# liuQuan98/GCL

Measured on AMD Instinct MI355X. Metric: active voxels/sec thru ResUNetBN2C fwd+bwd+GCL loss, KITTI 0.3m, higher is better.
Workload: dtype f32; 1 GPU; configs[2]: GCL training step (finest_contrastive_loss), ResUNetBN2C-32 conv1 k=5, KITTI-shaped ray-cast clouds @0.3 m, bs=4 x 7 clouds per GPU, positive groups 'fixed16'; global_batch=4, parallelism=dp1

## Files before the change

gcl_amd/MinkowskiEngine/native.py:

```python
import ctypes
import os
import threading

import torch
from torch.autograd.function import once_differentiable

from .. import _lib

PLAN_ENABLED = os.environ.get("GCL_PLAN", "1") == "1"
AUX_STREAM = {"0": "", "1": "1", "low": "low", "high": "high"}[os.environ.get("GCL_PLAN_AUX", "low")]


def _addr(t):
    return t.data_ptr() if t is not None else 0


_SIDE_STREAMS = {}


def eval_side_stream(device, n_rows=None):
    if os.environ.get("GCL_EVAL_SPLIT_MAPS", "1") == "0":
        return None
    if n_rows is not None and n_rows < int(os.environ.get("GCL_EVAL_SPLIT_MIN_ROWS", "100000")):
        return None
# ... 127 lines not shown
        if not self.handle:
            raise ValueError(lib.gcl_last_error().decode())
        self.handle = ctypes.c_void_p(self.handle)
        self._state = None
        self._key = None
        self.grad_targets = None
        self.bucket_of_param = None
        self.on_bucket = None
        self._param_ptrs = self._bn_ptrs = None
        self._ptr_key = None
        self.profile_next = False
        self.last_profile = None
        self._anchor = None
        self._aux = None
        self._eval_key = None

    def __del__(self):
        h, self.handle = getattr(self, "handle", None), None
        if h:
            try:
                _lib.load().gcl_plan_destroy(h)
            except Exception:
                pass

    @classmethod
    def from_tape(cls, tape, model, x_in, in_level, spec_keys):
        from . import ops
        if ops.PRECISION != "fp16x3" or not ops.FUSE_GRAD_ADD:
            raise ValueError("the plan runs the default arithmetic (fp16x3, fused gradient adds) only")
        params = [p for p in model.parameters()]
# ... 217 lines not shown
        for i, r in enumerate(self.records):
            for k in ("w", "bias", "bn_w", "bn_b"):
                p = r[k]
                if p >= 0 and p in self.bucket_of_param:
                    b = self.bucket_of_param[p]
                    lowest[b] = min(lowest.get(b, i), i)
        cuts = sorted(set(lowest.values()), reverse=True)
        segs, hi = [], n
        for c in cuts:
            segs.append((c, hi, sorted(b for b, i in lowest.items() if i == c)))
            hi = c
        if hi > 0:
            segs.append((0, hi, []))
        return segs

    def _backward(self, run, dy):
        lib = _lib.load()
        targets = run.grad_targets
        flat = None
        if targets is None:
            sizes = [p.numel() for p in self.params]
            flat = torch.empty(sum(sizes), dtype=torch.float32, device=dy.device)
            targets, off = [], 0
            for p, s in zip(self.params, sizes):
                targets.append(flat[off:off + s].view_as(p))
                off += s
        gp = (ctypes.c_void_p * len(targets))(*[t.data_ptr() for t in targets])
        st = _lib.stream()
        for first, last, buckets in run.segments:
            _lib.check(lib.gcl_plan_backward(self.handle, _lib.ptr(run.arena), _lib.ptr(dy, torch.float32), gp, first,
                                             last, st), "gcl_plan_backward")
            for b in buckets:
                self.on_bucket(b)
        if self.profile_next:
            self.profile_next = False
            self._profile_pending = True
            lib.gcl_plan_profile(self.handle, 0)
        run.done = True
        run.arena = run.maps = run.y = run.x = None
        return None if flat is None else targets

    def profile_records(self):
        lib = _lib.load()
        buf = (ctypes.c_double * (8 * 1024))()
        n = lib.gcl_plan_profile_read(self.handle, buf, 1024)
        return [tuple(buf[8 * i + j] for j in range(8)) for i in range(max(0, n))]
```

gcl_amd/_lib.py:

```python
import ctypes
import os
import subprocess

import torch

_HERE = os.path.dirname(os.path.abspath(__file__))
CSRC = os.path.join(_HERE, "csrc")
LIB_PATH = os.environ.get("GCL_LIB_PATH", os.path.join(CSRC, "libgcl_hip.so"))
SOURCES = ["coords.hip", "conv.hip", "norm.hip", "loss.hip", "pairloss.hip", "data.hip", "sc2pcr.hip", "plan.hip", "match.hip", "ransac.hip", "regstats.hip", "fpfh.hip",
           "valpose.hip", "pairmatch.hip", "icp.hip"]
HEADER = os.path.join(os.path.dirname(_HERE), "include", "gcl_amd.h")

_vp, _i32, _i64, _f32 = ctypes.c_void_p, ctypes.c_int32, ctypes.c_int64, ctypes.c_float
_f64 = ctypes.c_double

MAX_LEVELS, MAX_MAPS = 8, 16
MAPS_PINNED_BYTES = 512 * (MAX_MAPS + 1)
ERR_ARENA = -4


class MapSpec(ctypes.Structure):
    _fields_ = [("t_in", _i32), ("kernel_size", _i32), ("stride", _i32), ("tables", _i32), ("pairs", _i32)]


# ... 105 lines not shown
    "gcl_col_sum": (_i32, [_vp, _i64, _i32, _vp, _vp, _vp]),
    "gcl_maps_arena_bytes": (_i64, [_i64, _vp, _i32, _i32]),
    "gcl_maps_build": (_i32, [_vp, _i64, _vp, _i32, _i32, _vp, _i64, _vp, _vp, _vp]),
    "gcl_maps_build_split": (_i32, [_vp, _i64, _vp, _i32, _i32, _vp, _i64, _vp, _vp, _vp, _vp]),
    "gcl_plan_create": (_vp, [_vp, _i32, _i32, _i32, _vp, _i32, _i32]),
    "gcl_plan_destroy": (None, [_vp]),
    "gcl_plan_state_bytes": (_i64, [_vp]),
    "gcl_plan_arena_bytes": (_i64, [_vp, _vp]),
    "gcl_plan_forward": (_i32, [_vp, _vp, _vp, _vp, _vp, _vp, _vp, _i64, _vp, _vp]),
    "gcl_plan_eval_state_bytes": (_i64, [_vp]),
    "gcl_plan_eval_arena_bytes": (_i64, [_vp, _vp]),
    "gcl_plan_forward_eval": (_i32, [_vp, _vp, _vp, _vp, _vp, _i32, _vp, _vp, _i64, _vp, _vp]),
    "gcl_plan_backward": (_i32, [_vp, _vp, _vp, _vp, _i32, _i32, _vp]),
    "gcl_plan_release": (_i32, [_vp, _vp]),
    "gcl_plan_set_aux_stream": (_i32, [_vp, _vp]),
    "gcl_stream_create_cu_share": (_i32, [_i32, _i32, ctypes.POINTER(ctypes.c_void_p)]),
    "gcl_stream_destroy": (_i32, [_vp]),
    "gcl_plan_profile": (_i32, [_vp, _i32]),
    "gcl_plan_profile_read": (_i32, [_vp, _vp, _i32]),
    "gcl_sc2_chunks": (_i32, []),
    "gcl_sc2_refine_partial_len": (_i32, []),
    "gcl_sc2_confidence": (_i32, [_vp, _vp, _i32, _f32, _i32, _vp, _vp, _vp, _vp]),
    "gcl_sc2_confidence_scratch_bytes": (_i64, [_i32]),
    "gcl_sc2_confidence_sparse": (_i32, [_vp, _vp, _i32, _f32, _i32, _vp, _vp, _vp, _vp, _vp]),
    "gcl_sc2_register_scratch_bytes": (_i64, [_i32]),
    "gcl_sc2_register": (_i32, [_vp, _vp, _i32, _f32, _i32, _f32, _i32, _i32, _i32, _f32, _f32, _i32, _vp, _vp, _vp, _vp, _vp,
                                _vp, _vp, _vp, _vp, _vp]),
    "gcl_sc2_register_batch_scratch_bytes": (_i64, [_i32, _i32]),
    "gcl_sc2_register_batch": (_i32, [_vp, _vp, _i32, _i32, _vp, _vp, _f32, _i32, _f32, _i32, _i32, _f32, _f32, _i32, _vp, _vp,
                                      _vp, _vp, _vp, _vp, _vp, _vp, _vp, _vp]),
# ... 163 lines not shown
```

gcl_amd/csrc/plan.hip:

```cpp
#include "common.h"

#include <string.h>

#include <new>
#include <utility>
#include <vector>

namespace gcl {

__device__ __forceinline__ float amax4p(float m, const float4& v) {
  return fmaxf(m, fmaxf(fmaxf(fabsf(v.x), fabsf(v.y)), fmaxf(fabsf(v.z), fabsf(v.w))));
}
__device__ __forceinline__ void publish_amax_wg(float m, int* slot) {
#pragma unroll
  for (int o = 32; o > 0; o >>= 1) m = fmaxf(m, __shfl_xor(m, o));
  __shared__ float wm[4];
  if ((threadIdx.x & 63) == 0) wm[threadIdx.x >> 6] = m;
  __syncthreads();
  if (threadIdx.x == 0)
    amax_slot_publish(slot, __float_as_int(fmaxf(fmaxf(wm[0], wm[1]), fmaxf(wm[2], wm[3]))), blockIdx.x);
}

__global__ void __launch_bounds__(256) k_relu_fwd(const float4* __restrict__ x, long long n4, float4* __restrict__ y,
                                                  int* amax) {
// ... 66 lines not shown
    const int q = (int)(i - r * c4);
    float4 u = reinterpret_cast<const float4*>(a + r * a_ld)[q];
    if (b) {
      const float4 v = reinterpret_cast<const float4*>(b + r * b_ld)[q];
      u = make_float4(u.x + v.x, u.y + v.y, u.z + v.z, u.w + v.w);
    }
    y[i] = u;
  }
}
__global__ void __launch_bounds__(256) k_add2(const float4* __restrict__ a, const float4* __restrict__ b, long long n4,
                                              float4* __restrict__ y) {
  for (long long i = (long long)blockIdx.x * 256 + threadIdx.x; i < n4; i += (long long)gridDim.x * 256) {
    const float4 u = a[i], v = b[i];
    y[i] = make_float4(u.x + v.x, u.y + v.y, u.z + v.z, u.w + v.w);
  }
}
__global__ void __launch_bounds__(256) k_identity_pairs(int* __restrict__ p, long long n, long long total) {
  long long i = (long long)blockIdx.x * 256 + threadIdx.x;
  if (i < total) p[i] = i < n ? (int)i : -1;
}

void fill32(void* p, long long n_words, unsigned v, hipStream_t st);
void tables_fill(int64_t* tables, long long slots, int32_t* zero4, hipStream_t st);
int coords_insert_impl(const int32_t* coords, int64_t n, int64_t* table, int64_t cap, int32_t* status, bool table_ready,
                       void* stream);
int stride_map_impl(const int32_t* coords_in, int64_t n_in, const int32_t* n_in_dev, int32_t t_out, int64_t* table_out,
                    int64_t cap_out, int32_t* scratch, int32_t* coords_out, int32_t* n_out_dev, int32_t* status,
                    int64_t* index_out, bool table_ready, void* stream);

static inline unsigned grid_for(long long items, unsigned cap = 4096) {
// ... 284 lines not shown
  std::vector<long long> wK, wcin, wcout, off_fwd, off_bwd;
  long long bytes_fwd = 0, bytes_bwd = 0, wgs_fwd = 0, wgs_bwd = 0;
  int n_bwd = 0;
  std::vector<char> made;
  std::vector<char> fuse_relu;
  std::vector<int> cat_left;
  std::vector<int> mask_from;
  std::vector<long long> host_tables, uploaded;
  bool eval = false;
  void* const* bn_eval = nullptr;
  bool eval_repack = true;
  hipStream_t aux = nullptr;
  std::vector<hipEvent_t> events;
  size_t events_used = 0;
  bool aux_dirty = false;
  bool profile = false;
  std::vector<ProfRec> prof;
  size_t prof_used = 0;
};

static long long state_words(const Plan& P) { return (long long)P.worder.size() * (2 + 8 + 8); }

static int32_t* new_slot(Plan& P) {
  if (P.next_slot >= P.n_slots) {
    P.slots_exhausted = true;
    return P.slot_pool;
  }
  return P.slot_pool + (P.next_slot++) * GCL_AMAX_WORDS;
}

// ... 492 lines not shown
    float* scratch = A.take_n<float>(gcl_conv_bwd_weight_scratch_len(op.K, op.cin, op.cout, m.seg_off[op.K], n_sorted));
    const bool pl = pl_w;
    ProfScope ps(P, ws, 2, pairs, op.cin, op.cout, n_in, n_out, op.K);
    const int32_t* rgb = (sorted_side != 0 && n_sorted == m.n_out) ? m.dw_bounds : nullptr;
    PLAN_CALL(gcl_conv_bwd_weight_rg(pl ? (const float*)x.planes : x.ptr, n_in, pl ? (const float*)dy.planes : dy.ptr, n_out,
                                     pl ? 1 : 0, sorted_side, pa, pb, m.seg_off, op.K, op.cin, op.cout, 4, P.saved[i].x_amax,
                                     dy.amax, scratch, dW, rgb, (void*)ws));
  }
  if (op.bias >= 0) {
    double* scratch = A.take_n<double>(gcl_bn_scratch_len(n_out, op.cout));
    PLAN_CALL(gcl_col_sum(dy.ptr, n_out, op.cout, scratch, (float*)grads[op.bias], (void*)ws));
  }
  return GCL_OK;
}

static int plan_backward(Plan& P, const float* dy, void* const* grads, int first, int last, hipStream_t st) {
  Arena& A = P.A;
  const gcl_maps_desc& M = *P.maps;
  const size_t nw = P.worder.size();
  if (last == (int)P.ops.size()) {
    P.g[P.ops.back().y] = TState();
    P.g[P.ops.back().y].ptr = (float*)dy;
  }
  if (P.bwd_packed && last == (int)P.ops.size()) {
    int rcj = join_aux(P, st);
    if (rcj) return rcj;
  }
  if (!P.bwd_packed) {
    P.pack_bwd = (unsigned char*)A.take(P.bytes_bwd);
    if (P.n_bwd && !A.dry) {
      const long long* tab = (const long long*)P.state;
      PLAN_CALL(gcl_pack_weights_multi((const int64_t*)(tab + 2 * nw + 8 * nw), P.n_bwd, P.wgs_bwd, 4, P.w_amax, P.pack_bwd,
                                       (void*)st));
    }
    P.bwd_packed = true;
  }
  for (int i = last - 1; i >= first; --i) {
    const gcl_plan_op& op = P.ops[i];
    const long long n_out = M.n_rows[op.level_out], n_in = M.n_rows[op.level_in];
    TState g = P.g[op.y];
    P.g[op.y] = TState();
    if (!g.ptr) continue;
    int rc;
    switch (op.kind) {
      case GCL_OP_CONVBN: {
        const OpSaved& sv = P.saved[i];
        const int c = op.cout;
        float* sum_g = (float*)grads[op.bn_b];
        float* sum_gx = (float*)grads[op.bn_w];
        double* scratch = A.take_n<double>(gcl_bn_scratch_len(n_out, c));
        const bool bound = sv.xrange && c >= P.presplit && !is_stem(op, M.maps[op.map]);
        TState d;
// ... 40 lines not shown
        if ((rc = give(P, op.x2, g.ptr + ca, n_out * cb, st, nullptr, op.cout, cb))) return rc;
        break;
      }
      case GCL_OP_ROWNORM: {
        if ((rc = contiguous(P, g, n_out, op.cout, st))) return rc;
        float* dx = A.take_n<float>(n_in * op.cin);
        int32_t* slot = new_slot(P);
        PLAN_CALL(gcl_row_normalize_bwd(P.t[op.y].ptr, g.ptr, P.saved[i].norm, n_out, op.cout, dx, slot, (void*)st));
        if ((rc = give(P, op.x, dx, n_in * op.cin, st, slot, 0, op.cin))) return rc;
        break;
      }
      default:
        return GCL_ERR_ARG;
    }
  }
  return join_aux(P, st);
}

static int check_maps(const Plan& P, const gcl_maps_desc* M) {
  GCL_CHECK_ARG(M && M->n_levels >= 1 && M->n_levels <= GCL_MAX_LEVELS && M->n_maps >= 0 && M->n_maps <= GCL_MAX_MAPS,
                "gcl_plan: bad maps descriptor");
  for (size_t i = 0; i < P.ops.size(); ++i) {
    const gcl_plan_op& op = P.ops[i];
    GCL_CHECK_ARG(op.level_in < M->n_levels && op.level_out < M->n_levels, "gcl_plan: record %d uses a level the maps lack", (int)i);
    if (op.kind == GCL_OP_CONVBN || op.kind == GCL_OP_CONV) {
      GCL_CHECK_ARG(op.map >= 0 && op.map < M->n_maps, "gcl_plan: record %d names map %d of %d", (int)i, op.map, M->n_maps);
      const gcl_map_desc& m = M->maps[op.map];
      GCL_CHECK_ARG(m.K == op.K, "gcl_plan: record %d expects K = %d, map %d has %d", (int)i, op.K, op.map, m.K);
      const int lin = op.transpose ? m.level_out : m.level_in, lout = op.transpose ? m.level_in : m.level_out;
      GCL_CHECK_ARG(lin == op.level_in && lout == op.level_out, "gcl_plan: record %d and map %d disagree on the levels", (int)i, op.map);
// ... 135 lines not shown
  for (size_t i = 0; ok && i < P->ops.size(); ++i) {
    const gcl_plan_op& a = P->ops[i];
    if ((a.kind != GCL_OP_CONV && a.kind != GCL_OP_CONVBN) || a.cin <= 4 || a.x == 0) continue;
    int r = -1, consumers = 0;
    for (size_t j = 0; j < P->ops.size(); ++j) {
      if (P->ops[j].kind == GCL_OP_RELU && P->ops[j].y == a.x) r = (int)j;
      consumers += (P->ops[j].x == a.x) + (P->ops[j].x2 == a.x);
    }
    if (r >= 0 && consumers == 1 && a.x != P->ops.back().y) P->mask_from[i] = r;
  }
  if (!ok) {
    set_error("gcl_plan_create: malformed or unsupported operator records");
    delete P;
    return nullptr;
  }
  for (size_t q = 0; q < nw; ++q) {
    if (!P->wK[q]) {
      set_error("gcl_plan_create: weight_order names a parameter no record uses");
      delete P;
      return nullptr;
    }
    const long long bytes = (gcl_pack_weights_bytes((int)P->wK[q], (int)P->wcin[q], (int)P->wcout[q], 4) + 255) / 256 * 256;
    P->off_fwd[q] = P->bytes_fwd;
    P->bytes_fwd += bytes;
    if (P->wmode[q]) {
      P->off_bwd[q] = P->bytes_bwd;
      P->bytes_bwd += bytes;
      ++P->n_bwd;
    }
  }
// ... 158 lines not shown
  bool found = false;
  for (PassState* q : P->passes)
    if (q->forward_done && q->key == arena) found = true;
  if (found && P->aux && P->aux_dirty) {
    GCL_CHECK_HIP(hipStreamSynchronize(P->aux));
    P->aux_dirty = false;
  }
  for (PassState* q : P->passes)
    if (q->forward_done && q->key == arena) *q = PassState();
  return GCL_OK;
}

int gcl_plan_backward(void* plan, void* arena, const float* dy, void* const* grads_host, int32_t first_op,
                      int32_t last_op, void* stream) {
  Plan* P = (Plan*)plan;
  GCL_CHECK_ARG(P && grads_host, "gcl_plan_backward: null pointer");
  PassState* slot = nullptr;
  for (PassState* q : P->passes)
    if (q->forward_done && q->key == arena) slot = q;
  GCL_CHECK_ARG(slot, "gcl_plan_backward: no forward pass to differentiate in this arena");
  GCL_CHECK_ARG(first_op >= 0 && first_op < last_op && last_op <= (int)P->ops.size(), "gcl_plan_backward: bad record range");
  GCL_CHECK_ARG(last_op != (int)P->ops.size() || dy, "gcl_plan_backward: the last segment needs dy");
  static_cast<PassState&>(*P) = std::move(*slot);
  P->maps = &P->maps_copy;
  int rc = plan_backward(*P, dy, grads_host, first_op, last_op, (hipStream_t)stream);
  if (rc == GCL_OK && !P->A.fits()) {
    set_error("gcl_plan_backward: arena overrun");
    rc = GCL_ERR_ARENA;
  }
  if (rc == GCL_OK && P->slots_exhausted) {
    set_error("gcl_plan_backward: amax slot pool exhausted");
    rc = GCL_ERR_ARG;
  }
  if (first_op == 0 || rc != GCL_OK) P->forward_done = false;
  *slot = std::move(static_cast<PassState&>(*P));
  slot->maps = &slot->maps_copy;
  static_cast<PassState&>(*P) = PassState();
  return rc;
}

int gcl_plan_set_aux_stream(void* plan, void* stream) {
  Plan* P = (Plan*)plan;
  GCL_CHECK_ARG(P, "gcl_plan_set_aux_stream: null plan");
  P->aux = (hipStream_t)stream;
  return GCL_OK;
}

int gcl_stream_create_cu_share(int32_t percent, int32_t low_priority, void** stream_out) {
  GCL_CHECK_ARG(stream_out && percent >= 1 && percent <= 100, "gcl_stream_create_cu_share: percent must be 1..100");
  int dev = 0;
  hipDeviceProp_t prop;
  GCL_CHECK_HIP(hipGetDevice(&dev));
  GCL_CHECK_HIP(hipGetDeviceProperties(&prop, dev));
  const int n_cu = prop.multiProcessorCount, words = (n_cu + 31) / 32;
  int on = (int)((long long)n_cu * percent / 100);
  if (on < 8) on = 8;
  std::vector<uint32_t> mask((size_t)words, 0u);
  for (int i = 0; i < on && i < n_cu; ++i) mask[(size_t)i >> 5] |= 1u << (i & 31);
  hipStream_t st = nullptr;
// ... 34 lines not shown
```

gcl_amd/lib/colocation_trainer.py:

```python
import os
import types

import numpy as np
import torch
from torch.autograd.function import once_differentiable

import gcl_amd.MinkowskiEngine as ME
from gcl_amd import _lib
from gcl_amd.model import load_model

DEFAULT_CONFIG = dict(
    model="ResUNetBN2C", model_n_out=32, conv1_kernel_size=5, normalize_feature=True, bn_momentum=0.05,
    optimizer="SGD", lr=0.1, momentum=0.8, weight_decay=1e-4, exp_gamma=0.99,
    batch_size=4, num_pos_per_batch=256, num_hn_samples_per_batch=256, iter_size=1,
    hit_ratio_thresh=0.3, val_max_iter=400, nn_max_n=500,
    pos_thresh=0.1, neg_thresh=1.4, finest_thresh=0.2, pos_weight=1.0, neg_weight=1.0, finest_weight=1.0,
    square_loss=True, block_finest_gradient=False, use_hard_negative=True, use_pair_group_positive_loss=False,
    use_group_circle_loss=False, safe_radius=0.75, voxel_size=0.3,
    triplet_num_pos=256, triplet_num_hn=512, triplet_num_rand=1024,
)


def make_config(**overrides):
    cfg = dict(DEFAULT_CONFIG)
    cfg.update(overrides)
    return types.SimpleNamespace(**cfg)


class _GCLLossFn(torch.autograd.Function):

    @staticmethod
    def forward(ctx, F, index, goff, flag, sel, sel1, sel2, pos_thresh, fin_thresh, neg_thresh, flags=0,
                pairpos=None):
        lib = _lib.require_gpu()
        F = F.contiguous()
        n, c = F.shape
        dev = F.device
        n_sel, m = sel.shape[0], sel1.shape[0]
        pos = torch.empty(n_sel, dtype=torch.float32, device=dev)
        fin = torch.empty(n_sel, dtype=torch.float32, device=dev)
        st = _lib.stream()
# ... 10 lines not shown
                                     _lib.ptr(sel2, torch.int64), m, c, 1, _lib.ptr(nn_scratch), _lib.ptr(dmin),
                                     _lib.ptr(arg), st), "gcl_nn_rowmin")
        cap = 64
        while cap < 2 * m:
            cap *= 2
        table = torch.empty((cap, 2), dtype=torch.int64, device=dev)
        keep = torch.empty(m, dtype=torch.uint8, device=dev)
        _lib.check(lib.gcl_neg_mask(_lib.ptr(sel1), _lib.ptr(sel2), _lib.ptr(arg), m, _lib.ptr(index), _lib.ptr(goff),
                                    goff.shape[0] - 1, index.shape[0], _lib.ptr(table), cap, _lib.ptr(keep), st),
                   "gcl_neg_mask")
        out = torch.empty(2, dtype=torch.float32, device=dev)
        _lib.check(lib.gcl_neg_loss_fwd(_lib.ptr(dmin), _lib.ptr(keep), m, neg_thresh, _lib.ptr(out), st),
                   "gcl_neg_loss_fwd")
        ctx.save_for_backward(F, index, goff, flag, sel, sel1, sel2, dmin, arg, keep, out, pairpos)
        ctx.th = (pos_thresh, fin_thresh, neg_thresh, int(flags))
        return pos, fin, out[0]

    @staticmethod
    @once_differentiable
    def backward(ctx, gpos, gfin, gneg):
        return (_GCLLossFn.backward_terms(ctx, gpos, gfin, gneg),) + (None,) * 11

    @staticmethod
    def backward_terms(ctx, gpos, gfin, gneg):
        lib = _lib.load()
        F, index, goff, flag, sel, sel1, sel2, dmin, arg, keep, out, pairpos = ctx.saved_tensors
        pos_thresh, fin_thresh, neg_thresh, flags = ctx.th
        n, c = F.shape
        st = _lib.stream()
        dF = torch.zeros_like(F)
        gpos_c, gfin_c = gpos.contiguous(), gfin.contiguous()
        _lib.check(lib.gcl_group_loss_bwd(_lib.ptr(F), c, _lib.ptr(index), _lib.ptr(goff), _lib.ptr(flag),
                                          _lib.ptr(sel), sel.shape[0], pos_thresh, fin_thresh, flags,
                                          _lib.ptr(pairpos), _lib.ptr(gpos_c), _lib.ptr(gfin_c), _lib.ptr(dF), st),
                   "gcl_group_loss_bwd")
        g = gneg.reshape(1).contiguous()
        _lib.check(lib.gcl_neg_loss_bwd(_lib.ptr(F), c, _lib.ptr(sel1), _lib.ptr(sel2), _lib.ptr(arg), _lib.ptr(dmin),
                                        _lib.ptr(keep), sel1.shape[0], neg_thresh, _lib.ptr(out), _lib.ptr(g),
                                        _lib.ptr(dF), st), "gcl_neg_loss_bwd")
        return dF


class _GCLTotalLossFn(torch.autograd.Function):

    @staticmethod
    def forward(ctx, F, index, goff, flag, sel, sel1, sel2, pos_thresh, fin_thresh, neg_thresh, flags, pairpos,
                w_pos, w_fin, w_neg):
        lib = _lib.require_gpu()
        pos, fin, neg = _GCLLossFn.forward(ctx, F, index, goff, flag, sel, sel1, sel2, pos_thresh, fin_thresh, neg_thresh,
                                           flags, pairpos)
        out = torch.empty(4, dtype=torch.float32, device=F.device)
        _lib.check(lib.gcl_loss_combine(_lib.ptr(pos), _lib.ptr(fin), pos.shape[0], _lib.ptr(neg), float(w_pos),
                                        float(w_fin), float(w_neg), _lib.ptr(out), _lib.stream()), "gcl_loss_combine")
        ctx.w = (float(w_pos), float(w_fin), float(w_neg))
# ... 381 lines not shown
        fuse = (fused_total and not cfg.use_group_circle_loss and cfg.finest_weight != 0 and cfg.use_hard_negative
                and os.environ.get("GCL_FUSED_LOSS_TOTAL", "1") == "1")
        terms = self.location_loss(
            F_out, input_dict["group"], input_dict["index"], input_dict.get("index_hash"), input_dict["finest_flag"],
            max_pos_cluster=cfg.num_pos_per_batch * cfg.batch_size,
            max_hn_samples=cfg.num_hn_samples_per_batch * cfg.batch_size,
            points=input_dict["sinput_C"][:, 1:] if cfg.use_group_circle_loss else None,
            batch_lengths=input_dict.get("batch_lengths"), draws=draws, prepared=input_dict.get("_loss_inputs"),
            total_weights=(self.pos_weight, self.finest_weight, self.neg_weight) if fuse else None)
        if len(terms) == 4:
            return terms[0], tuple(terms[1:]), F_out
        pos, fin, neg = terms
        loss = self.pos_weight * pos + self.finest_weight * fin + self.neg_weight * neg
        return loss, (pos, fin, neg), F_out

    def _draw_for(self, input_dict):
        cfg = self.config
        if cfg.use_group_circle_loss:
            sizes = torch.as_tensor(input_dict["group"]).cpu().numpy() if cfg.use_pair_group_positive_loss else None
            return draw_circle_selections(len(input_dict["group"]), cfg.num_pos_per_batch * cfg.batch_size, sizes,
                                          cfg.use_pair_group_positive_loss)
        sizes = None
        if cfg.use_pair_group_positive_loss:
            sizes = torch.as_tensor(input_dict["group"]).cpu().numpy()
        return draw_selections(len(input_dict["group"]), len(input_dict["sinput_C"]),
                               cfg.num_pos_per_batch * cfg.batch_size, cfg.num_hn_samples_per_batch * cfg.batch_size,
                               sizes, cfg.use_pair_group_positive_loss, random_negative=not cfg.use_hard_negative)

    def _prefetch_maps(self, batch):
        C = batch.get("sinput_C") if isinstance(batch, dict) else None
# ... 177 lines not shown
                if not np.isnan(rre):
                    rre_meter.update(rre)
                hit_ratio = self.evaluate_hit_ratio(xyz0_corr, xyz1_corr, T_gt,
                                                    thresh=getattr(self.config, "hit_ratio_thresh", 0.3))
                hit_ratio_meter.update(hit_ratio)
                feat_match_ratio.update(float(hit_ratio > 0.05))
                num_data += 1
        return {"loss": loss_meter.avg, "rre": rre_meter.avg, "rte": rte_meter.avg,
                "feat_match_ratio": feat_match_ratio.avg, "hit_ratio": hit_ratio_meter.avg, "n": num_data}

    def train_step(self, input_dict, draws=None):
        with torch.cuda.device(self.device):
            return self._train_step(input_dict, draws)

    def _train_step(self, input_dict, draws=None):
        self.model.train()
        micro = list(input_dict) if isinstance(input_dict, (list, tuple)) else [input_dict]
        n_micro = len(micro)
        if draws is None:
            mdraws = [self._draw_for(b) for b in micro]
        else:
            mdraws = list(draws) if isinstance(input_dict, (list, tuple)) else [draws]
        plan = self._plan_for_step(micro)
        if plan is not None:
            self._seat_gradients()
        elif self.ddp is not None:
            self.ddp.flat_grad.zero_()
        else:
            if os.environ.get("GCL_ZERO_NONE", "1") == "1":
                for p in self._params:
                    p.grad = None
            else:
                self.optimizer.zero_grad(set_to_none=False)
        tot_loss, tot_parts, n_rows = None, None, 0
        for i, (b, d) in enumerate(zip(micro, mdraws)):
            if self.ddp is not None:
                self.ddp.set_last_microstep(i == n_micro - 1)
            if plan is not None:
                plan.grad_targets = self._grad_views if i == 0 else self._grad_views2
                overlap = self.ddp is not None and n_micro == 1 and self.ddp.overlap and self.ddp.world > 1
                plan.bucket_of_param = self._plan_buckets() if overlap else None
                plan.on_bucket = self.ddp.bucket_ready if overlap else None
            wait_for_batch(b)
            try:
                loss, parts, F_out = self.forward_loss(b, d, fused_total=(n_micro == 1))
                if n_micro > 1:
                    parts = tuple(p / n_micro for p in parts)
                    loss = self.pos_weight * parts[0] + self.finest_weight * parts[1] + self.neg_weight * parts[2]
                loss.backward()
            finally:
                if plan is not None:
                    plan.grad_targets = plan.bucket_of_param = plan.on_bucket = None
            if plan is not None and i > 0:
                self._flat_grad.add_(self._flat_grad2)
            release_batch(b)
            n_rows += F_out.shape[0]
            dl, dp = loss.detach(), tuple(p.detach() for p in parts)
            tot_loss = dl if tot_loss is None else tot_loss + dl
            tot_parts = dp if tot_parts is None else tuple(a + b_ for a, b_ in zip(tot_parts, dp))
        if self.ddp is not None:
            self.ddp.all_reduce_gradients()
        self.optimizer.step()
        return tot_loss, tot_parts, n_rows


def prefetch_to_device(batches, device, keys=("sinput_C", "sinput_F", "group", "index", "finest_flag"), ring=4):
# ... 10 lines not shown
            copy_stream.wait_event(slot["free"])
        slot["busy"], slot["age"], slot["free"] = True, i, None
        with torch.cuda.stream(copy_stream):
            for k in keys:
                v = b.get(k)
                if isinstance(v, torch.Tensor) and not v.is_cuda:
                    if not v.is_pinned():
                        v = v.pin_memory()
                    n = v.numel()
                    buf = slot["bufs"].get(k)
                    if buf is None or buf.dtype != v.dtype or buf.numel() < n:
                        buf = slot["bufs"][k] = torch.empty(int(n * 1.25) + 16, dtype=v.dtype, device=dev)
                    dst = buf[:n].view(v.shape)
                    dst.copy_(v, non_blocking=True)
                    out[k] = dst
            ev = torch.cuda.Event()
            ev.record(copy_stream)
        out["_h2d_event"], out["_h2d_slot"] = ev, (slot, i)
        yield out


def release_batch(batch):
    ar = batch.get("_map_arena") if isinstance(batch, dict) else None
    if ar is not None and ar["busy"]:
        ev = torch.cuda.Event()
        ev.record(torch.cuda.current_stream())
        with ar["lock"]:
            ar["free"], ar["busy"] = ev, False
    st = batch.get("_h2d_slot") if isinstance(batch, dict) else None
    if st is None:
# ... 25 lines not shown
```

include/gcl_amd.h:

```cpp
#ifndef GCL_AMD_H
#define GCL_AMD_H

#include <stdint.h>

#ifdef __cplusplus
extern "C" {
#endif

#define GCL_OK 0
#define GCL_ERR_ARG (-1)
#define GCL_ERR_HIP (-2)
#define GCL_ERR_NO_DEVICE (-3)

#define GCL_PAIR_CHUNK 128

const char* gcl_last_error(void);
int gcl_version(void);
int gcl_device_count(void);

int gcl_coords_insert(const int32_t* coords, int64_t n, int64_t* table, int64_t cap,
                      int32_t* status, void* stream);

int64_t gcl_scan_scratch_len(int64_t n);
int gcl_stride_map(const int32_t* coords_in, int64_t n_in, const int32_t* n_in_dev, int32_t t_out,
// ... 357 lines not shown
void gcl_plan_destroy(void* plan);
int64_t gcl_plan_state_bytes(const void* plan);
int64_t gcl_plan_arena_bytes(void* plan, const gcl_maps_desc* maps_host);
int gcl_plan_forward(void* plan, const gcl_maps_desc* maps_host, const float* x, void* const* params_host,
                     void* const* bn_stats_host, void* state, void* arena, int64_t arena_bytes, float** y_out_host,
                     void* stream);
int64_t gcl_plan_eval_state_bytes(const void* plan);
int64_t gcl_plan_eval_arena_bytes(void* plan, const gcl_maps_desc* maps_host);
int gcl_plan_forward_eval(void* plan, const gcl_maps_desc* maps_host, const float* x, void* const* params_host,
                          void* const* bn_eval_host, int32_t repack, void* state, void* arena, int64_t arena_bytes,
                          float** y_out_host, void* stream);
int gcl_plan_backward(void* plan, void* arena, const float* dy, void* const* grads_host, int32_t first_op,
                      int32_t last_op, void* stream);
int gcl_plan_release(void* plan, void* arena);
int gcl_plan_set_aux_stream(void* plan, void* stream);
int gcl_stream_create_cu_share(int32_t percent, int32_t low_priority, void** stream_out);
int gcl_stream_destroy(void* stream);
int gcl_plan_profile(void* plan, int32_t enable);
int gcl_plan_profile_read(void* plan, double* records_host, int32_t max_records);

int gcl_col_sum(const float* x, int64_t n, int32_t c, double* scratch, float* out, void* stream);

int gcl_pair_key_table(const int64_t* pos_pairs, int64_t n_pos, int64_t seed, int64_t* table, int64_t cap, void* stream);
int gcl_pair_key_mask(const int64_t* ap, int32_t col, const int64_t* b, const int32_t* b_arg, int64_t nb, int32_t m,
                      int64_t seed, const int64_t* table, int64_t cap, int64_t* b_out, uint8_t* keep, void* stream);
#define GCL_TRIPLET_OUT 20
int64_t gcl_triplet_scratch_len(int32_t m);
int gcl_triplet_fwd(const float* f0, int64_t n0, const float* f1, int64_t n1, int32_t c, const int64_t* ap,
                    const int64_t* neg, const uint8_t* tag, const uint8_t* keep, int32_t m, float margin, float* work,
                    float* out, void* stream);
// ... 49 lines not shown
```

Measured before the change: 46.02 million active voxels/s.

## Run tail backward only on loss-touched rows via gather/scatter suffix path

The loss backward now records which output rows actually receive gradient (rows in the sampled positive groups and the hard-negative pairs). The plan backward uses that list to run the row-local suffix of the network (final 1x1 convs, ReLUs, row normalisation) on a compacted set of rows: it gathers activations, runs backward on the compacted rows, then scatters the result into a zeroed full gradient. This removes dense work over all rows for the tail layers. In exchange it adds gather, scatter, memset, scan and dry-run arena sizing work, and it relies on the touched-row capacity computed on the host.

```diff
diff --git a/gcl_amd/MinkowskiEngine/native.py b/gcl_amd/MinkowskiEngine/native.py
--- a/gcl_amd/MinkowskiEngine/native.py
+++ b/gcl_amd/MinkowskiEngine/native.py
@@ -165,6 +165,7 @@
         self._anchor = None
         self._aux = None
         self._eval_key = None
+        self._touched = None
 
     def __del__(self):
         h, self.handle = getattr(self, "handle", None), None
@@ -412,6 +413,26 @@
             segs.append((0, hi, []))
         return segs
 
+    def set_touched_rows(self, rows, cap):
+        lib = _lib.load()
+        self._touched = rows
+        _lib.check(lib.gcl_plan_set_touched_rows(self.handle, _lib.ptr(rows, torch.int32), int(cap)),
+                   "gcl_plan_set_touched_rows")
+
+    def touch_loss_rows(self, index, goff, sel, rows_a, rows_b, n_rows, cap):
+        lib = _lib.load()
+        dev = index.device
+        scratch = torch.empty(int(lib.gcl_touched_rows_scratch_len(int(n_rows))), dtype=torch.int32, device=dev)
+        out = torch.empty(int(cap) + 1, dtype=torch.int32, device=dev)
+        rows, count = out[:cap], out[cap:]
+        _lib.check(lib.gcl_touched_rows(_lib.ptr(index, torch.int64), index.shape[0], _lib.ptr(goff, torch.int64),
+                                        goff.shape[0] - 1, _lib.ptr(sel, torch.int64), sel.shape[0],
+                                        _lib.ptr(rows_a, torch.int64), rows_a.shape[0], _lib.ptr(rows_b, torch.int64),
+                                        rows_b.shape[0], int(n_rows), _lib.ptr(scratch), _lib.ptr(rows), int(cap),
+                                        _lib.ptr(count), _lib.stream()), "gcl_touched_rows")
+        self.set_touched_rows(rows, cap)
+        return rows, count
+
     def _backward(self, run, dy):
         lib = _lib.load()
         targets = run.grad_targets
@@ -430,6 +451,7 @@
                                              last, st), "gcl_plan_backward")
             for b in buckets:
                 self.on_bucket(b)
+        self._touched = None
         if self.profile_next:
             self.profile_next = False
             self._profile_pending = True
diff --git a/gcl_amd/_lib.py b/gcl_amd/_lib.py
--- a/gcl_amd/_lib.py
+++ b/gcl_amd/_lib.py
@@ -143,6 +143,13 @@
     "gcl_plan_backward": (_i32, [_vp, _vp, _vp, _vp, _i32, _i32, _vp]),
     "gcl_plan_release": (_i32, [_vp, _vp]),
     "gcl_plan_set_aux_stream": (_i32, [_vp, _vp]),
+    "gcl_plan_touched_suffix": (_i32, [_vp]),
+    "gcl_plan_set_touched_rows": (_i32, [_vp, _vp, _i64]),
+    "gcl_plan_suffix_rows_used": (_i64, [_vp]),
+    "gcl_gather_rows": (_i32, [_vp, _i32, _i64, _vp, _i64, _i32, _f32, _vp, _vp]),
+    "gcl_scatter_rows": (_i32, [_vp, _vp, _i64, _i32, _i64, _vp, _i32, _vp]),
+    "gcl_touched_rows_scratch_len": (_i64, [_i64]),
+    "gcl_touched_rows": (_i32, [_vp, _i64, _vp, _i64, _vp, _i32, _vp, _i32, _vp, _i32, _i64, _vp, _vp, _i64, _vp, _vp]),
     "gcl_stream_create_cu_share": (_i32, [_i32, _i32, ctypes.POINTER(ctypes.c_void_p)]),
     "gcl_stream_destroy": (_i32, [_vp]),
     "gcl_plan_profile": (_i32, [_vp, _i32]),
diff --git a/gcl_amd/csrc/plan.hip b/gcl_amd/csrc/plan.hip
--- a/gcl_amd/csrc/plan.hip
+++ b/gcl_amd/csrc/plan.hip
@@ -104,6 +104,64 @@
     const float4 u = a[i], v = b[i];
     y[i] = make_float4(u.x + v.x, u.y + v.y, u.z + v.z, u.w + v.w);
   }
+}
+template <typename V>
+__device__ __forceinline__ V splat(float v);
+template <>
+__device__ __forceinline__ float splat<float>(float v) { return v; }
+template <>
+__device__ __forceinline__ float4 splat<float4>(float v) { return make_float4(v, v, v, v); }
+template <typename V>
+__global__ void __launch_bounds__(256) k_gather_rows(const float* __restrict__ src, int ld, long long n_src,
+                                                     const int* __restrict__ rows, long long cap, int cv, float pad,
+                                                     V* __restrict__ out) {
+  const long long total = cap * cv;
+  for (long long i = (long long)blockIdx.x * 256 + threadIdx.x; i < total; i += (long long)gridDim.x * 256) {
+    const long long j = i / cv;
+    const int q = (int)(i - j * cv);
+    const long long r = rows[j];
+    out[i] = (r >= 0 && r < n_src) ? reinterpret_cast<const V*>(src + r * ld)[q] : splat<V>(pad);
+  }
+}
+__global__ void __launch_bounds__(256) k_scatter_rows(const float4* __restrict__ src, const int* __restrict__ rows,
+                                                      long long cap, int c4, long long n_dst, float* __restrict__ dst,
+                                                      int ld) {
+  const long long total = cap * c4;
+  for (long long i = (long long)blockIdx.x * 256 + threadIdx.x; i < total; i += (long long)gridDim.x * 256) {
+    const long long j = i / c4;
+    const int q = (int)(i - j * c4);
+    const long long r = rows[j];
+    if (r >= 0 && r < n_dst) reinterpret_cast<float4*>(dst + r * ld)[q] = src[i];
+  }
+}
+__global__ void __launch_bounds__(256) k_touch_rows(const long long* __restrict__ ids, long long count, long long n,
+                                                    int* __restrict__ flag) {
+  const long long i = (long long)blockIdx.x * 256 + threadIdx.x;
+  if (i >= count) return;
+  const long long r = ids[i];
+  if (r >= 0 && r < n) flag[r] = 1;
+}
+__global__ void __launch_bounds__(64) k_touch_groups(const long long* __restrict__ index, long long n_index,
+                                                     const long long* __restrict__ goff, long long n_groups,
+                                                     const long long* __restrict__ sel, long long n,
+                                                     int* __restrict__ flag) {
+  const long long g = sel[blockIdx.x];
+  if (g < 0 || g >= n_groups) return;
+  long long b = goff[g], e = goff[g + 1];
+  if (b < 0) b = 0;
+  if (e > n_index) e = n_index;
+  for (long long j = b + threadIdx.x; j < e; j += 64) {
+    const long long r = index[j];
+    if (r >= 0 && r < n) flag[r] = 1;
+  }
+}
+__global__ void __launch_bounds__(256) k_touch_emit(const int* __restrict__ flag, const int* __restrict__ pos, long long n,
+                                                    int* __restrict__ rows, long long cap, int* __restrict__ n_touched) {
+  const long long i = (long long)blockIdx.x * 256 + threadIdx.x;
+  const int total = pos[n - 1] + flag[n - 1];
+  if (i == 0) *n_touched = total;
+  if (i < n && flag[i] && pos[i] < cap) rows[pos[i]] = (int)i;
+  if (i < cap && i >= total) rows[i] = -1;
 }
 __global__ void __launch_bounds__(256) k_identity_pairs(int* __restrict__ p, long long n, long long total) {
   long long i = (long long)blockIdx.x * 256 + threadIdx.x;
@@ -418,6 +476,11 @@
   std::vector<hipEvent_t> events;
   size_t events_used = 0;
   bool aux_dirty = false;
+  int suffix_first = 0;
+  bool suffix_rows_ok = false;
+  const int32_t* touched = nullptr;
+  long long touched_cap = 0;
+  long long suffix_rows_used = 0;
   bool profile = false;
   std::vector<ProfRec> prof;
   size_t prof_used = 0;
@@ -940,10 +1003,110 @@
   return GCL_OK;
 }
 
-static int plan_backward(Plan& P, const float* dy, void* const* grads, int first, int last, hipStream_t st) {
+static int suffix_backward(Plan& P, const float* dy, void* const* grads, const int32_t* rows, long long cap, TState* g_out,
+                           hipStream_t st) {
+  Arena& A = P.A;
+  const gcl_maps_desc& M = *P.maps;
+  const int n_ops = (int)P.ops.size();
+  const long long n = M.n_rows[P.ops.back().level_out];
+  std::vector<std::pair<const float*, float*>> gathered;
+  auto gather = [&](const float* src, int ld, int c, float pad) -> float* {
+    for (auto& e : gathered)
+      if (e.first == src) return e.second;
+    float* out = A.take_n<float>(cap * c);
+    if (!A.dry && gcl_gather_rows(src, ld, n, rows, cap, c, pad, out, (void*)st) != GCL_OK) return nullptr;
+    gathered.push_back({src, out});
+    return out;
+  };
+  std::vector<char> masked(P.ops.size(), 0);
+  TState g;
+  g.ptr = gather(dy, P.ops.back().cout, P.ops.back().cout, 0.f);
+  if (!g.ptr) return GCL_ERR_ARG;
+  int rc;
+  for (int i = n_ops - 1; i >= P.suffix_first && g.ptr; --i) {
+    const gcl_plan_op& op = P.ops[i];
+    switch (op.kind) {
+      case GCL_OP_ROWNORM: {
+        const float* y = gather(P.t[op.y].ptr, op.cout, op.cout, 0.f);
+        const float* norm = gather(P.saved[i].norm, 1, 1, 1.f);
+        float* dx = A.take_n<float>(cap * op.cin);
+        int32_t* slot = new_slot(P);
+        PLAN_CALL(gcl_row_normalize_bwd(y, g.ptr, norm, cap, op.cout, dx, slot, (void*)st));
+        g = TState();
+        g.ptr = dx;
+        g.amax = slot;
+        break;
+      }
+      case GCL_OP_RELU: {
+        if (masked[i]) break;
+        const float* y = gather(P.t[op.y].ptr, P.t[op.y].ld ? P.t[op.y].ld : op.cout, op.cout, 0.f);
+        const long long numel = cap * op.cout;
+        float* gx = A.take_n<float>(numel);
+        int32_t* slot = new_slot(P);
+        if (!A.dry) {
+          hipLaunchKernelGGL(k_relu_bwd, dim3(grid_for(numel / 4)), dim3(256), 0, st, (const float4*)g.ptr, (const float4*)y,
+                             numel / 4, (float4*)gx, slot);
+          GCL_CHECK_LAUNCH();
+        }
+        g = TState();
+        g.ptr = gx;
+        g.amax = slot;
+        break;
+      }
+      case GCL_OP_CONV: {
+        const TState& x = P.t[op.x];
+        const int wi = P.widx[op.w];
+        if ((rc = ensure_amax(P, g, cap * op.cout, st))) return rc;
+        const int32_t* w_amax = P.w_amax + (long long)wi * GCL_AMAX_WORDS;
+        const bool pl = op.cout >= P.presplit;
+        if (pl && P.made[op.x] && (rc = ensure_planes(P, g, cap, op.cout, st))) return rc;
+        const float* xc = gather(x.ptr, x.ld ? x.ld : op.cin, op.cin, 0.f);
+        if (!A.dry) GCL_CHECK_LAUNCH();
+        hipStream_t ws = fork_aux(P, st);
+        TState d;
+        if (P.made[op.x]) {
+          GCL_CHECK_ARG(P.wmode[wi] == 1, "gcl_plan_backward: record %d: input-gradient pack mode mismatch", i);
+          d.ptr = A.take_n<float>(cap * op.cin);
+          ProfScope ps(P, st, 0, (double)cap, op.cout, op.cin, cap, cap, op.K);
+          if (P.mask_from[i] >= 0) {
+            d.amax = new_slot(P);
+            PLAN_CALL(gcl_conv_fwd_fused(pl ? (const float*)g.planes : g.ptr, cap, pl ? 1 : 0, P.pack_bwd + P.off_bwd[wi], 4,
+                                         g.amax, w_amax, nullptr, nullptr, nullptr, cap, op.K, op.cout, op.cin, nullptr, nullptr,
+                                         xc, 2, d.amax, d.ptr, nullptr, 0, (void*)st));
+            masked[P.mask_from[i]] = 1;
+          } else
+            PLAN_CALL(gcl_conv_fwd(pl ? (const float*)g.planes : g.ptr, cap, pl ? 1 : 0, P.pack_bwd + P.off_bwd[wi], 4, g.amax,
+                                   w_amax, nullptr, nullptr, nullptr, cap, op.K, op.cout, op.cin, nullptr, d.ptr, nullptr, 0,
+                                   (void*)st));
+        }
+        {
+          float* scratch = A.take_n<float>(gcl_conv_bwd_weight_rows_scratch_len(op.cin, op.cout, 4, cap));
+          ProfScope ps(P, ws, 3, (double)cap, op.cin, op.cout, cap, cap, op.K);
+          PLAN_CALL(gcl_conv_bwd_weight_rows(xc, g.ptr, cap, op.cin, op.cout, 4, P.saved[i].x_amax, g.amax, scratch,
+                                             (float*)grads[op.w], (void*)ws));
+        }
+        if (op.bias >= 0) {
+          double* scratch = A.take_n<double>(gcl_bn_scratch_len(cap, op.cout));
+          PLAN_CALL(gcl_col_sum(g.ptr, cap, op.cout, scratch, (float*)grads[op.bias], (void*)ws));
+        }
+        g = d;
+        break;
+      }
+      default:
+        return GCL_ERR_ARG;
+    }
+  }
+  if (!A.dry) GCL_CHECK_LAUNCH();
+  *g_out = g;
+  return GCL_OK;
+}
+
+static int plan_backward(Plan& P, const float* dy, void* const* grads, int first, int last, hipStream_t st,
+                         const int32_t* rows = nullptr, long long cap = 0) {
   Arena& A = P.A;
   const gcl_maps_desc& M = *P.maps;
   const size_t nw = P.worder.size();
+  const int n_ops = (int)P.ops.size();
   if (last == (int)P.ops.size()) {
     P.g[P.ops.back().y] = TState();
     P.g[P.ops.back().y].ptr = (float*)dy;
@@ -961,7 +1124,49 @@
     }
     P.bwd_packed = true;
   }
-  for (int i = last - 1; i >= first; --i) {
+  int top = last - 1;
+  long long reserve_to = 0;
+  if (last == n_ops && !A.dry) P.suffix_rows_used = 0;
+  if (last == n_ops && P.suffix_first < n_ops && P.suffix_rows_ok && first <= P.suffix_first) {
+    const gcl_plan_op& head = P.ops[P.suffix_first];
+    const long long n = M.n_rows[head.level_in];
+    const long long off0 = A.off, slot0 = P.next_slot;
+    if (A.dry) {
+      TState g;
+      const long long cap_max = (n - 1) / 2;
+      if (cap_max > 0) {
+        int rc = suffix_backward(P, dy, grads, nullptr, cap_max, &g, st);
+        if (rc) return rc;
+        A.take_n<float>(n * head.cin);
+        reserve_to = A.off;
+        A.off = off0;
+        P.next_slot = slot0;
+      }
+    } else if (rows && cap > 0 && 2 * cap < n) {
+      TState g;
+      A.dry = true;
+      int rc = suffix_backward(P, dy, grads, rows, cap, &g, st);
+      A.take_n<float>(n * head.cin);
+      const bool fits = rc == GCL_OK && A.off <= A.size;
+      A.dry = false;
+      A.off = off0;
+      P.next_slot = slot0;
+      if (fits) {
+        if ((rc = suffix_backward(P, dy, grads, rows, cap, &g, st))) return rc;
+        P.g[P.ops.back().y] = TState();
+        if (g.ptr) {
+          float* dx = A.take_n<float>(n * head.cin);
+          GCL_CHECK_HIP(hipMemsetAsync(dx, 0, (size_t)(n * head.cin) * sizeof(float), st));
+          if ((rc = gcl_scatter_rows(g.ptr, rows, cap, head.cin, n, dx, head.cin, (void*)st))) return rc;
+          if ((rc = give(P, head.x, dx, n * head.cin, st, g.amax, 0, head.cin))) return rc;
+        }
+        top = P.suffix_first - 1;
+        P.suffix_rows_used = cap;
+      }
+    }
+  }
+  for (int i = top; i >= first; --i) {
+    if (reserve_to && i == P.suffix_first - 1 && A.off < reserve_to) A.off = reserve_to;
     const gcl_plan_op& op = P.ops[i];
     const long long n_out = M.n_rows[op.level_out], n_in = M.n_rows[op.level_in];
     TState g = P.g[op.y];
@@ -1032,6 +1237,7 @@
         return GCL_ERR_ARG;
     }
   }
+  if (reserve_to && A.off < reserve_to) A.off = reserve_to;
   return join_aux(P, st);
 }
 
@@ -1197,6 +1403,27 @@
     delete P;
     return nullptr;
   }
+  {
+    auto consumers = [&](int t) {
+      int c = 0;
+      for (const gcl_plan_op& o : P->ops) c += (o.x == t) + (o.x2 == t);
+      return c;
+    };
+    auto row_local = [](const gcl_plan_op& o) {
+      return o.kind == GCL_OP_ROWNORM || o.kind == GCL_OP_RELU ||
+             (o.kind == GCL_OP_CONV && o.K == 1 && !o.transpose && o.level_in == o.level_out && o.cin > 4);
+    };
+    int s = n_ops;
+    while (s > 0 && row_local(P->ops[s - 1]) &&
+           (s == n_ops || (P->ops[s].x == P->ops[s - 1].y && consumers(P->ops[s - 1].y) == 1)))
+      --s;
+    while (s < n_ops && consumers(P->ops[s].x) != 1) ++s;
+    P->suffix_first = s;
+    P->suffix_rows_ok = true;
+    for (int i = s; i < n_ops; ++i)
+      if (P->ops[i].kind == GCL_OP_CONV && gcl_conv_bwd_weight_rows_scratch_len(P->ops[i].cin, P->ops[i].cout, 4, 128) <= 0)
+        P->suffix_rows_ok = false;
+  }
   for (size_t q = 0; q < nw; ++q) {
     if (!P->wK[q]) {
       set_error("gcl_plan_create: weight_order names a parameter no record uses");
@@ -1385,7 +1612,12 @@
 int gcl_plan_backward(void* plan, void* arena, const float* dy, void* const* grads_host, int32_t first_op,
                       int32_t last_op, void* stream) {
   Plan* P = (Plan*)plan;
-  GCL_CHECK_ARG(P && grads_host, "gcl_plan_backward: null pointer");
+  GCL_CHECK_ARG(P, "gcl_plan_backward: null pointer");
+  const int32_t* rows = P->touched;
+  const long long cap = P->touched_cap;
+  P->touched = nullptr;
+  P->touched_cap = 0;
+  GCL_CHECK_ARG(grads_host, "gcl_plan_backward: null pointer");
   PassState* slot = nullptr;
   for (PassState* q : P->passes)
     if (q->forward_done && q->key == arena) slot = q;
@@ -1394,7 +1626,7 @@
   GCL_CHECK_ARG(last_op != (int)P->ops.size() || dy, "gcl_plan_backward: the last segment needs dy");
   static_cast<PassState&>(*P) = std::move(*slot);
   P->maps = &P->maps_copy;
-  int rc = plan_backward(*P, dy, grads_host, first_op, last_op, (hipStream_t)stream);
+  int rc = plan_backward(*P, dy, grads_host, first_op, last_op, (hipStream_t)stream, rows, cap);
   if (rc == GCL_OK && !P->A.fits()) {
     set_error("gcl_plan_backward: arena overrun");
     rc = GCL_ERR_ARENA;
@@ -1414,6 +1646,82 @@
   Plan* P = (Plan*)plan;
   GCL_CHECK_ARG(P, "gcl_plan_set_aux_stream: null plan");
   P->aux = (hipStream_t)stream;
+  return GCL_OK;
+}
+
+int gcl_plan_touched_suffix(const void* plan) {
+  if (!plan) return -1;
+  return ((const Plan*)plan)->suffix_first;
+}
+
+int gcl_gather_rows(const float* src, int32_t ld, int64_t n_src, const int32_t* rows, int64_t cap, int32_t c, float pad,
+                    float* out, void* stream) {
+  GCL_CHECK_ARG(src && rows && out && n_src > 0 && cap > 0 && c > 0 && ld >= c, "gcl_gather_rows: bad argument");
+  const bool vec = c % 4 == 0 && ld % 4 == 0 && (((uintptr_t)src | (uintptr_t)out) & 15) == 0;
+  if (vec)
+    hipLaunchKernelGGL(k_gather_rows<float4>, dim3(grid_for(cap * c / 4)), dim3(256), 0, (hipStream_t)stream, src, ld,
+                       (long long)n_src, (const int*)rows, (long long)cap, c / 4, pad, (float4*)out);
+  else
+    hipLaunchKernelGGL(k_gather_rows<float>, dim3(grid_for(cap * c)), dim3(256), 0, (hipStream_t)stream, src, ld,
+                       (long long)n_src, (const int*)rows, (long long)cap, c, pad, out);
+  GCL_CHECK_LAUNCH();
+  return GCL_OK;
+}
+
+int gcl_scatter_rows(const float* src, const int32_t* rows, int64_t cap, int32_t c, int64_t n_dst, float* dst, int32_t ld,
+                     void* stream) {
+  GCL_CHECK_ARG(src && rows && dst && n_dst > 0 && cap > 0, "gcl_scatter_rows: bad argument");
+  GCL_CHECK_ARG(c > 0 && c % 4 == 0 && ld >= c && ld % 4 == 0 && (((uintptr_t)src | (uintptr_t)dst) & 15) == 0,
+                "gcl_scatter_rows: channel count and row pitch must be multiples of 4, the tensors 16-byte aligned");
+  hipLaunchKernelGGL(k_scatter_rows, dim3(grid_for(cap * c / 4)), dim3(256), 0, (hipStream_t)stream, (const float4*)src,
+                     (const int*)rows, (long long)cap, c / 4, (long long)n_dst, dst, ld);
+  GCL_CHECK_LAUNCH();
+  return GCL_OK;
+}
+
+int64_t gcl_plan_suffix_rows_used(const void* plan) {
+  if (!plan) return -1;
+  return ((const Plan*)plan)->suffix_rows_used;
+}
+
+int gcl_plan_set_touched_rows(void* plan, const int32_t* rows, int64_t cap) {
+  Plan* P = (Plan*)plan;
+  GCL_CHECK_ARG(P, "gcl_plan_set_touched_rows: null plan");
+  GCL_CHECK_ARG((rows && cap > 0) || (!rows && cap == 0), "gcl_plan_set_touched_rows: a list needs a positive length");
+  P->touched = rows;
+  P->touched_cap = cap;
+  return GCL_OK;
+}
+
+int64_t gcl_touched_rows_scratch_len(int64_t n_rows) { return n_rows > 0 ? gcl_scan_scratch_len(n_rows) : 0; }
+
+int gcl_touched_rows(const int64_t* index, int64_t n_index, const int64_t* goff, int64_t n_groups, const int64_t* sel,
+                     int32_t n_sel, const int64_t* rows_a, int32_t n_a, const int64_t* rows_b, int32_t n_b, int64_t n_rows,
+                     int32_t* scratch, int32_t* rows, int64_t cap, int32_t* n_touched, void* stream) {
+  GCL_CHECK_ARG(scratch && rows && n_touched && n_rows > 0 && n_rows < (1ll << 31) && cap > 0,
+                "gcl_touched_rows: bad argument");
+  GCL_CHECK_ARG(n_sel >= 0 && n_a >= 0 && n_b >= 0 && n_index >= 0 && n_groups >= 0, "gcl_touched_rows: negative count");
+  GCL_CHECK_ARG(n_sel == 0 || (index && goff && sel), "gcl_touched_rows: group selections need index, goff and sel");
+  GCL_CHECK_ARG((n_a == 0 || rows_a) && (n_b == 0 || rows_b), "gcl_touched_rows: null row array");
+  hipStream_t st = (hipStream_t)stream;
+  int32_t *flag = scratch, *pos = scratch + n_rows, *bs = scratch + 2 * n_rows;
+  GCL_CHECK_HIP(hipMemsetAsync(flag, 0, (size_t)n_rows * sizeof(int32_t), st));
+  if (n_sel)
+    hipLaunchKernelGGL(k_touch_groups, dim3((unsigned)n_sel), dim3(64), 0, st, (const long long*)index, (long long)n_index,
+                       (const long long*)goff, (long long)n_groups, (const long long*)sel, (long long)n_rows, flag);
+  if (n_a)
+    hipLaunchKernelGGL(k_touch_rows, dim3((unsigned)cdiv(n_a, 256)), dim3(256), 0, st, (const long long*)rows_a, (long long)n_a,
+                       (long long)n_rows, flag);
+  if (n_b)
+    hipLaunchKernelGGL(k_touch_rows, dim3((unsigned)cdiv(n_b, 256)), dim3(256), 0, st, (const long long*)rows_b, (long long)n_b,
+                       (long long)n_rows, flag);
+  GCL_CHECK_LAUNCH();
+  int rc = gcl_exclusive_scan_i32(flag, n_rows, pos, bs, stream);
+  if (rc) return rc;
+  const long long items = n_rows > cap ? n_rows : cap;
+  hipLaunchKernelGGL(k_touch_emit, dim3((unsigned)cdiv(items, 256)), dim3(256), 0, st, (const int*)flag, (const int*)pos,
+                     (long long)n_rows, rows, (long long)cap, n_touched);
+  GCL_CHECK_LAUNCH();
   return GCL_OK;
 }
 
diff --git a/gcl_amd/lib/colocation_trainer.py b/gcl_amd/lib/colocation_trainer.py
--- a/gcl_amd/lib/colocation_trainer.py
+++ b/gcl_amd/lib/colocation_trainer.py
@@ -25,6 +25,9 @@
     cfg = dict(DEFAULT_CONFIG)
     cfg.update(overrides)
     return types.SimpleNamespace(**cfg)
+
+
+_TOUCHED_REQUEST = None
 
 
 class _GCLLossFn(torch.autograd.Function):
@@ -65,6 +68,7 @@
                    "gcl_neg_loss_fwd")
         ctx.save_for_backward(F, index, goff, flag, sel, sel1, sel2, dmin, arg, keep, out, pairpos)
         ctx.th = (pos_thresh, fin_thresh, neg_thresh, int(flags))
+        ctx.touched = _TOUCHED_REQUEST
         return pos, fin, out[0]
 
     @staticmethod
@@ -89,6 +93,9 @@
         _lib.check(lib.gcl_neg_loss_bwd(_lib.ptr(F), c, _lib.ptr(sel1), _lib.ptr(sel2), _lib.ptr(arg), _lib.ptr(dmin),
                                         _lib.ptr(keep), sel1.shape[0], neg_thresh, _lib.ptr(out), _lib.ptr(g),
                                         _lib.ptr(dF), st), "gcl_neg_loss_bwd")
+        req, ctx.touched = getattr(ctx, "touched", None), None
+        if req is not None:
+            req[0].touch_loss_rows(index, goff, sel, sel1, sel2, n, req[1])
         return dF
 
 
@@ -500,6 +507,18 @@
         loss = self.pos_weight * pos + self.finest_weight * fin + self.neg_weight * neg
         return loss, (pos, fin, neg), F_out
 
+    def _touched_cap(self, input_dict, draws):
+        if self.config.use_group_circle_loss or draws is None:
+            return None
+        sizes = input_dict.get("_group_host", input_dict["group"])
+        if isinstance(sizes, torch.Tensor):
+            if sizes.is_cuda:
+                return None
+            sizes = sizes.numpy()
+        pos_sel, sel_hn1, sel_hn2 = draws[:3]
+        cap = int(np.asarray(sizes)[np.asarray(pos_sel)].sum()) + len(sel_hn1) + len(sel_hn2)
+        return (cap + 127) // 128 * 128
+
     def _draw_for(self, input_dict):
         cfg = self.config
         if cfg.use_group_circle_loss:
@@ -707,6 +726,7 @@
             return self._train_step(input_dict, draws)
 
     def _train_step(self, input_dict, draws=None):
+        global _TOUCHED_REQUEST
         self.model.train()
         micro = list(input_dict) if isinstance(input_dict, (list, tuple)) else [input_dict]
         n_micro = len(micro)
@@ -736,13 +756,18 @@
                 plan.on_bucket = self.ddp.bucket_ready if overlap else None
             wait_for_batch(b)
             try:
+                cap = self._touched_cap(b, d) if plan is not None else None
+                _TOUCHED_REQUEST = (plan, cap) if cap else None
                 loss, parts, F_out = self.forward_loss(b, d, fused_total=(n_micro == 1))
+                _TOUCHED_REQUEST = None
                 if n_micro > 1:
                     parts = tuple(p / n_micro for p in parts)
                     loss = self.pos_weight * parts[0] + self.finest_weight * parts[1] + self.neg_weight * parts[2]
                 loss.backward()
             finally:
+                _TOUCHED_REQUEST = None
                 if plan is not None:
+                    plan.set_touched_rows(None, 0)
                     plan.grad_targets = plan.bucket_of_param = plan.on_bucket = None
             if plan is not None and i > 0:
                 self._flat_grad.add_(self._flat_grad2)
@@ -783,6 +808,8 @@
                     dst = buf[:n].view(v.shape)
                     dst.copy_(v, non_blocking=True)
                     out[k] = dst
+                    if k == "group":
+                        out["_group_host"] = v
             ev = torch.cuda.Event()
             ev.record(copy_stream)
         out["_h2d_event"], out["_h2d_slot"] = ev, (slot, i)
diff --git a/include/gcl_amd.h b/include/gcl_amd.h
--- a/include/gcl_amd.h
+++ b/include/gcl_amd.h
@@ -395,6 +395,17 @@
                       int32_t last_op, void* stream);
 int gcl_plan_release(void* plan, void* arena);
 int gcl_plan_set_aux_stream(void* plan, void* stream);
+int gcl_plan_touched_suffix(const void* plan);
+int gcl_plan_set_touched_rows(void* plan, const int32_t* rows, int64_t cap);
+int64_t gcl_plan_suffix_rows_used(const void* plan);
+int64_t gcl_touched_rows_scratch_len(int64_t n_rows);
+int gcl_touched_rows(const int64_t* index, int64_t n_index, const int64_t* goff, int64_t n_groups, const int64_t* sel,
+                     int32_t n_sel, const int64_t* rows_a, int32_t n_a, const int64_t* rows_b, int32_t n_b, int64_t n_rows,
+                     int32_t* scratch, int32_t* rows, int64_t cap, int32_t* n_touched, void* stream);
+int gcl_gather_rows(const float* src, int32_t ld, int64_t n_src, const int32_t* rows, int64_t cap, int32_t c, float pad,
+                    float* out, void* stream);
+int gcl_scatter_rows(const float* src, const int32_t* rows, int64_t cap, int32_t c, int64_t n_dst, float* dst, int32_t ld,
+                     void* stream);
 int gcl_stream_create_cu_share(int32_t percent, int32_t low_priority, void** stream_out);
 int gcl_stream_destroy(void* stream);
 int gcl_plan_profile(void* plan, int32_t enable);
```

After: 46.63 million active voxels/s (median of 6 runs). 1.3% higher.
